# marekrams/tnac4o

Hardware: AMD Instinct MI355X
Metric: PEPS-contraction ms/sweep, chimera L=2048 chi=64 (boundary-MPS sweep _setup_rhoT) (lower is better)
Workload: dtype f64; 1 GPU; chimera L=2048 (Nx=Ny=16, Nc=8), synthetic couplings seed 20260004, beta=3, chi=64; one sweep = 16 rows of MPO absorb + compress_mps; one step = the sweeps of the 4 lattice rotations of one instance; parallelism=1 GPU: 4 lattice rotations of one instance interleaved on 4 HIP streams, mode=sweep

## Files before the change

include/tnpeps.h:

```cpp
#ifndef TNPEPS_H
#define TNPEPS_H
#include <stdint.h>

#ifdef __cplusplus
extern "C" {
#endif

int tn_version(void);
int tn_build_id(char* buf, int n);
int tn_stream_create_masked(const uint32_t* mask_host, int nwords, void** stream_out);
int tn_stream_destroy(void* stream);
int tn_last_error(char* buf, int n);

int tn_gemm(int64_t M, int64_t N, int64_t K, double alpha, const double* A, int64_t rsa, int64_t csa,
            const double* B, int64_t rsb, int64_t csb, double beta, double* C, int64_t rsc, int64_t csc,
            int64_t batch, int64_t bsa, int64_t bsb, int64_t bsc, void* ws, int64_t ws_bytes, void* stream);
int64_t tn_gemm_ws_bytes(int64_t M, int64_t N, int64_t K, int64_t batch);

int tn_factor_products_eligible(int64_t Z, int64_t I, int64_t J, int64_t K1, int64_t N, int64_t M, int first_batched);
int64_t tn_factor_products_ws_bytes(int64_t Z, int64_t I, int64_t J, int64_t K1, int64_t N, int first_batched);
int tn_factor_products(int64_t Z, int64_t I, int64_t J, int64_t K1, int64_t N, int64_t Mhi, int64_t Mlo, const double* P, int64_t pz,
                       int64_t pi, int64_t pk, const double* X, int64_t xk, int64_t xj, int64_t xn, const double* W, int64_t wm,
                       int64_t wq, double* Out, int64_t oz, int64_t ohi, int64_t olo, int64_t on, int first_batched, void* ws,
                       int64_t ws_bytes, void* stream);

int tn_absorb(const double* A, const double* W, double* out, int64_t Dl, int64_t pold, int64_t Dr, int64_t ba,
              int64_t po, int64_t bb, int64_t pi, int hconj, int64_t batch, int64_t bsA, int64_t bsW, int64_t bsOut,
              void* stream);

int tn_qr(double* A, int64_t rs, int64_t cs, int64_t m, int64_t n, double* Q, int64_t qrs, int64_t qcs, double* R,
          int64_t rrs, int64_t rcs, int nb, double rank_tol, int64_t* keff_host, void* ws, int64_t ws_bytes, void* stream);
int64_t tn_qr_ws_bytes(int64_t m, int64_t n, int nb);
int64_t tn_panel_orth_ws_bytes(int64_t nrows, int b);
int tn_panel_orth(const double* X, int64_t rs, int64_t cs, int64_t nrows, int b, double* Y, int64_t yrs, int64_t ycs, int method,
                  int* state9_host, double* dev_host, void* ws, int64_t ws_bytes, void* stream);
int tn_panel_stats(uint64_t* out16_host, int reset);
int tn_panel_stats_stream(uint64_t* out16_host, int reset, void* stream);
int tn_smallqr_stats(uint64_t* out4_host, int reset, void* stream);
int tn_fused_timeouts(int* count_host, void* stream);
int tn_qr_batched(double* A, int64_t rs, int64_t cs, int64_t m, int64_t n, double* Q, int64_t qrs, int64_t qcs, double* R,
// ... 198 lines not shown
```

tnac4o_amd/_lib.py:

```python
import ctypes as C
import os
import subprocess

HERE = os.path.dirname(os.path.abspath(__file__))
LIB_PATH = os.path.join(HERE, 'libtnpeps.so')
CSRC = os.path.join(HERE, 'csrc')
SOURCES = ['api.hip', 'gemm_f64.hip', 'rank_update.hip', 'factor_products.hip', 'small.hip', 'qr.hip', 'svd.hip', 'absorb.hip', 'misc.hip', 'beam.hip', 'prof.hip', 'cholqr.hip', 'smallqr.hip', 'fused.hip', 'peps.hip', 'env.hip', 'batch.hip', 'site.hip', 'chain.hip', 'beamsearch.hip', 'marginal.hip', 'sampler.hip', 'overlap.hip', 'relax.hip', 'exchange.hip', 'temper.hip', 'anneal.hip', 'rng.hip', 'droplets.hip', 'linkage.hip', 'lines.hip']

_i64, _f64, _int, _ptr = C.c_int64, C.c_double, C.c_int, C.c_void_p

SIGNATURES = {
    'tn_version': (_int, []),
    'tn_last_error': (_int, [C.c_char_p, _int]),
    'tn_build_id': (_int, [C.c_char_p, _int]),
    'tn_stream_create_masked': (_int, [C.POINTER(C.c_uint32), _int, C.POINTER(_ptr)]),
    'tn_stream_destroy': (_int, [_ptr]),
    'tn_gemm': (_int, [_i64, _i64, _i64, _f64, _ptr, _i64, _i64, _ptr, _i64, _i64, _f64, _ptr, _i64, _i64,
                       _i64, _i64, _i64, _i64, _ptr, _i64, _ptr]),
    'tn_gemm_ws_bytes': (_i64, [_i64, _i64, _i64, _i64]),
    'tn_factor_products_eligible': (_int, [_i64] * 6 + [_int]),
    'tn_factor_products_ws_bytes': (_i64, [_i64] * 5 + [_int]),
    'tn_factor_products': (_int, [_i64] * 7 + [_ptr, _i64, _i64, _i64, _ptr, _i64, _i64, _i64, _ptr, _i64, _i64, _ptr, _i64, _i64, _i64, _i64,
                                  _int, _ptr, _i64, _ptr]),
    'tn_absorb': (_int, [_ptr, _ptr, _ptr, _i64, _i64, _i64, _i64, _i64, _i64, _i64, _int, _i64, _i64, _i64, _i64, _ptr]),
    'tn_qr': (_int, [_ptr, _i64, _i64, _i64, _i64, _ptr, _i64, _i64, _ptr, _i64, _i64, _int, _f64, C.POINTER(_i64), _ptr, _i64,
              _ptr]),
    'tn_qr_ws_bytes': (_i64, [_i64, _i64, _int]),
    'tn_panel_orth_ws_bytes': (_i64, [_i64, _int]),
    'tn_panel_orth': (_int, [_ptr, _i64, _i64, _i64, _int, _ptr, _i64, _i64, _int, C.POINTER(_int), C.POINTER(_f64), _ptr, _i64, _ptr]),
    'tn_panel_stats': (_int, [C.POINTER(C.c_uint64), _int]),
    'tn_panel_stats_stream': (_int, [C.POINTER(C.c_uint64), _int, _ptr]),
    'tn_smallqr_stats': (_int, [C.POINTER(C.c_uint64), _int, _ptr]),
    'tn_fused_timeouts': (_int, [C.POINTER(_int), _ptr]),
    'tn_qr_batched': (_int, [_ptr, _i64, _i64, _i64, _i64, _ptr, _i64, _i64, _ptr, _i64, _i64, _int, _f64, C.POINTER(_i64), _i64, _i64, _i64,
                      _i64, _ptr, _i64, _ptr, C.POINTER(_ptr), _int]),
    'tn_svd_trunc': (_int, [_ptr, _i64, _i64, _i64, _i64, _i64, _f64, _ptr, _i64, _i64, _ptr, _ptr, _i64, _i64,
                            C.POINTER(_i64), C.POINTER(_f64), C.POINTER(_int), C.POINTER(_int), _ptr, _i64, _ptr]),
    'tn_svdvals': (_int, [_ptr, _i64, _i64, _i64, _i64, C.POINTER(_f64), C.POINTER(_int), C.POINTER(_int), _ptr, _i64,
                          _ptr]),
    'tn_svd_ws_bytes': (_i64, [_i64, _i64, _int]),
    'tn_svdvals_async': (_int, [_ptr, _i64, _i64, _i64, _i64, _ptr, _ptr]),
    'tn_svdvals_small_batched': (_int, [_ptr, _i64, _ptr, _ptr, _ptr]),
# ... 146 lines not shown
        objs = list(ex.map(one, SOURCES))
    cmd = [hipcc, '--offload-arch=gfx950', '-shared', '-fPIC', '-Wl,--no-undefined'] + os.environ.get('TN_EXTRA_HIPCC_FLAGS', '').split() + ['-o', LIB_PATH] + objs
    if verbose:
        print(' '.join(cmd), flush=True)
    subprocess.run(cmd, check=True)
    return LIB_PATH


def _stale(L):
    buf = C.create_string_buffer(64)
    L.tn_build_id.restype, L.tn_build_id.argtypes = _int, [C.c_char_p, _int]
    L.tn_build_id(buf, 64)
    return buf.value.decode() != source_hash()


SHORT_CALLS = ('tn_gemm', 'tn_gemm_ws_bytes', 'tn_qr_ws_bytes', 'tn_svd_ws_bytes', 'tn_absorb', 'tn_nfactor', 'tn_scale_by',
               'tn_normalize_pow2', 'tn_scale_phys', 'tn_calc_pn', 'tn_sample_pn', 'tn_score_pn', 'tn_nfactor_batched', 'tn_env_rr_batched', 'tn_env_rl_batched',
               'tn_balance', 'tn_merge_groups', 'tn_svdvals_async', 'tn_rar', 'tn_rar_ws_bytes', 'tn_env_mix', 'tn_env_mix_ws_bytes',
               'tn_apply_truncation', 'tn_apply_truncation_ws_bytes', 'tn_site_qr_ws_bytes', 'tn_gram_weights', 'tn_argsort_desc', 'tn_weighted_sum', 'tn_rows_norm2', 'tn_gather_scale_rows', 'tn_peps_factor', 'tn_mpo_from_factor', 'tn_env3', 'tn_env3_ws_bytes',
               'tn_cluster_marginal', 'tn_cluster_marginal_ws_bytes', 'tn_cluster_bond_marginal', 'tn_cluster_bond_marginal_ws_bytes',
               'tn_mpo_from_factor_ops', 'tn_env3_stack', 'tn_env3_stack_ws_bytes', 'tn_stack_cell_law', 'tn_stack_cell_law_ws_bytes',
               'tn_last_error')
_lib = None
ABI_VERSION = 25


def lib():
    global _lib
    if _lib is None:
        if not os.path.exists(LIB_PATH):
            raise RuntimeError('libtnpeps.so not found at %s: run `python -c "import __graft_entry__ as g; g.build()"` '
                               '(the HIP library is the only backend; there is no CPU fallback)' % LIB_PATH)
        L = C.CDLL(LIB_PATH)
        L.tn_version.restype = _int
        if not hasattr(L, 'tn_build_id') or (_stale(L) and not os.environ.get('TN_ALLOW_STALE_LIB')):
            raise RuntimeError('libtnpeps.so was built from other sources than csrc/*.hip + include/tnpeps.h in this tree: '
                               'rebuild it with `python -c "import __graft_entry__ as g; g.build()"` -- a stale library can '
                               'disagree with the ctypes signatures declared here')
        if L.tn_version() != ABI_VERSION:
            raise RuntimeError('libtnpeps.so implements C-ABI version %d, this package binds version %d: rebuild the library'
                               % (L.tn_version(), ABI_VERSION))
        if os.environ.get('TN_PYDLL', '1') != '0':
            P = C.PyDLL(LIB_PATH)
            for name in SHORT_CALLS:
                setattr(L, name, getattr(P, name))
            L._pydll = P
        for name, (res, args) in SIGNATURES.items():
# ... 16 lines not shown
```

tnac4o_amd/csrc/api.hip:

```cpp
#include <stdarg.h>

#include "../../include/tnpeps.h"
#include "common.h"

namespace tn {

static thread_local char g_err[512] = "";

void set_error(const char* fmt, ...) {
    va_list ap;
    va_start(ap, fmt);
    vsnprintf(g_err, sizeof(g_err), fmt, ap);
    va_end(ap);
}
const char* get_error() { return g_err; }

}

using namespace tn;
#define ST ((hipStream_t)stream)

extern "C" {

int tn_version(void) { return 25; }

#ifndef TN_SRC_HASH
#define TN_SRC_HASH "unknown"
#endif
int tn_build_id(char* buf, int n) {
    const char* e = TN_SRC_HASH;
    const int len = (int)strlen(e);
    if (buf && n > 0) {
        const int c = len < n - 1 ? len : n - 1;
        memcpy(buf, e, c);
        buf[c] = 0;
    }
    return len;
}

void tn_profile_enable(unsigned mask) { prof_set_mask(mask); }
void tn_profile_reset(void) { prof_reset(); }
void tn_profile_sample(unsigned every) { prof_set_sample(every); }
int tn_profile_get(int family, uint64_t* calls_host, double* ms_host, double* flops_host, double* bytes_host) {
    TN_CHECK_ARG(family >= 0 && family < PROF_NFAM, "unknown kernel family");
    TN_CHECK_ARG(calls_host && ms_host && flops_host && bytes_host, "null output");
    prof_get(-1, family, calls_host, ms_host, flops_host, bytes_host);
    return 0;
// ... 20 lines not shown
    const hipError_t e = hipStreamDestroy((hipStream_t)stream);
    return e == hipSuccess ? 0 : hip_fail(e, "hipStreamDestroy");
}

int tn_last_error(char* buf, int n) {
    const char* e = get_error();
    int len = (int)strlen(e);
    if (buf && n > 0) {
        int c = len < n - 1 ? len : n - 1;
        memcpy(buf, e, c);
        buf[c] = 0;
    }
    return len;
}

int tn_gemm(int64_t M, int64_t N, int64_t K, double alpha, const double* A, int64_t rsa, int64_t csa, const double* B,
            int64_t rsb, int64_t csb, double beta, double* C, int64_t rsc, int64_t csc, int64_t batch, int64_t bsa,
            int64_t bsb, int64_t bsc, void* ws, int64_t ws_bytes, void* stream) {
    TN_CHECK_ARG(M >= 0 && N >= 0 && K >= 0 && batch >= 0, "negative dimension");
    TN_CHECK_ARG(A && B && C, "null operand");
    return gemm(ST, M, N, K, alpha, A, rsa, csa, B, rsb, csb, beta, C, rsc, csc, batch, bsa, bsb, bsc, (double*)ws, ws_bytes);
}
int64_t tn_gemm_ws_bytes(int64_t M, int64_t N, int64_t K, int64_t batch) { return gemm_ws_bytes(M, N, K, batch); }

int tn_factor_products_eligible(int64_t Z, int64_t I, int64_t J, int64_t K1, int64_t N, int64_t M, int first_batched) {
    return factor_products_fits(Z, I, J, K1, N, M) && (first_batched || gemm_ws_bytes(Z * I, J * N, K1, 1) == 0) ? 1 : 0;
}
static int64_t factor_products_layout(char* base, int64_t Z, int64_t I, int64_t J, int64_t K1, int64_t N, int first_batched, double** S,
                                      double** gw, int64_t* gw_bytes) {
    WsCarve c{base};
    *gw_bytes = first_batched ? 0 : gemm_ws_bytes(Z * I, J * N, K1, 1);
    *S = c.take<double>(Z * I * J * N * 8);
    *gw = c.take<double>(*gw_bytes);
    return c.total();
}
int64_t tn_factor_products_ws_bytes(int64_t Z, int64_t I, int64_t J, int64_t K1, int64_t N, int first_batched) {
    double* S; double* gw; int64_t gb;
    return factor_products_layout(nullptr, Z, I, J, K1, N, first_batched, &S, &gw, &gb);
}
int tn_factor_products(int64_t Z, int64_t I, int64_t J, int64_t K1, int64_t N, int64_t Mhi, int64_t Mlo, const double* P, int64_t pz,
                       int64_t pi, int64_t pk, const double* X, int64_t xk, int64_t xj, int64_t xn, const double* W, int64_t wm,
                       int64_t wq, double* Out, int64_t oz, int64_t ohi, int64_t olo, int64_t on, int first_batched, void* ws,
                       int64_t ws_bytes, void* stream) {
    TN_CHECK_ARG(Z >= 1 && I >= 1 && J >= 1 && K1 >= 1 && N >= 1 && Mhi >= 1 && Mlo >= 1, "non-positive dimension");
    TN_CHECK_ARG(P && X && W && Out, "null operand");
    TN_CHECK_ARG((Z == 1 || pz == I * pi) && (first_batched || J == 1 || xj == N * xn), "the first product needs pz = I pi, and unbatched xj = N xn");
// ... 276 lines not shown
```

tnac4o_amd/csrc/common.h:

```cpp
#pragma once
#include <hip/hip_runtime.h>
#include <stdint.h>
#include <stdio.h>
#include <stdlib.h>
#include <string.h>

namespace tn {

void set_error(const char* fmt, ...);
const char* get_error();

inline int hip_fail(hipError_t e, const char* what) {
    set_error("%s: %s", what, hipGetErrorString(e));
    return (int)e > 0 ? (int)e : 1;
}

#define TN_CHECK_ARG(cond, msg)                \
    do {                                       \
        if (!(cond)) {                         \
            tn::set_error("%s: %s", __func__, msg); \
            return -1;                         \
        }                                      \
    } while (0)

// ... 63 lines not shown
void prof_note_qr(int64_t m, int64_t n, int64_t batch);
void prof_note_svd(int64_t k, int64_t n, int sweeps);
void prof_note_svdvals(int64_t k, int64_t n);
int prof_phase(int phase);
struct ProfPhase {
    int prev;
    explicit ProfPhase(int ph) : prev(prof_phase(ph)) {}
    ~ProfPhase() { prof_phase(prev); }
};
#define TN_PROF_LAUNCH(st, fam, launch) do { prof_begin(st, fam); launch; prof_end(st, fam, 0.0, 0.0); } while (0)
void prof_set_mask(unsigned mask);
void prof_set_sample(unsigned n);
void prof_reset();
void prof_get(int phase, int fam, uint64_t* calls, double* ms, double* flops, double* bytes);

struct Mat {
    double* p;
    int64_t rs, cs;
};
static inline Mat mat(double* p, int64_t rs, int64_t cs) { return Mat{p, rs, cs}; }
static inline Mat sub(Mat a, int64_t i, int64_t j) { return Mat{a.p + i * a.rs + j * a.cs, a.rs, a.cs}; }
static inline Mat tr(Mat a) { return Mat{a.p, a.cs, a.rs}; }

int gemm(hipStream_t st, int64_t M, int64_t N, int64_t K, double alpha, const double* A, int64_t rsa, int64_t csa,
         const double* B, int64_t rsb, int64_t csb, double beta, double* C, int64_t rsc, int64_t csc,
         int64_t batch = 1, int64_t bsa = 0, int64_t bsb = 0, int64_t bsc = 0, double* ws = nullptr,
         int64_t ws_bytes = 0);
int64_t gemm_ws_bytes(int64_t M, int64_t N, int64_t K, int64_t batch);
struct GemmExtra {
    const int* pairs = nullptr;
    const int* skip = nullptr;
    int pw = 0, mapA = 0, mapB = 0, mapC = 0;
    int force_splitk = 0;
    bool raw_partials = false;
    int* splitk_used = nullptr;
};
int gemm_forced_split(int64_t K, int s, int64_t* kchunk);
int gemm_ex(hipStream_t st, int64_t M, int64_t N, int64_t K, double alpha, const double* A, int64_t rsa, int64_t csa,
            const double* B, int64_t rsb, int64_t csb, double beta, double* C, int64_t rsc, int64_t csc, int64_t batch,
            int64_t bsa, int64_t bsb, int64_t bsc, double* ws, int64_t ws_bytes, const GemmExtra* x);

static inline int gemm(hipStream_t st, int64_t M, int64_t N, int64_t K, double alpha, Mat A, Mat B, double beta, Mat C,
                       double* ws = nullptr, int64_t ws_bytes = 0) {
    return gemm(st, M, N, K, alpha, A.p, A.rs, A.cs, B.p, B.rs, B.cs, beta, C.p, C.rs, C.cs, 1, 0, 0, 0, ws, ws_bytes);
}
int gemm_prof_family(int64_t M, int64_t N, int64_t K, int64_t rsc, int64_t csc);

int rank_update(hipStream_t st, int64_t m, int64_t n, int b, const double* W, int64_t wrs, int64_t wcs, const double* X, int64_t xrs,
                int64_t xcs, double* C, int64_t rsc, int64_t csc, const int* active);
static inline int rank_update(hipStream_t st, int64_t m, int64_t n, int b, Mat W, Mat X, Mat C, const int* active = nullptr) {
    return rank_update(st, m, n, b, W.p, W.rs, W.cs, X.p, X.rs, X.cs, C.p, C.rs, C.cs, active);
}

struct FactorProducts {
    int64_t Z, I, J, K1, N, Mhi, Mlo;
    const double* P; int64_t pz, pi, pk;
    const double* X; int64_t xk, xj, xn;
    const double* W; int64_t wm, wq;
    double* Out; int64_t oz, ohi, olo, on;
};
bool factor_products_fits(int64_t Z, int64_t I, int64_t J, int64_t K1, int64_t N, int64_t M);
inline bool factor_products_on() { return env_flag_on("TN_FACTOR_FUSED"); }
int factor_products(hipStream_t st, const FactorProducts& f);

constexpr int NBMAX = 64;

int gram_partial(hipStream_t st, const double* X, int64_t vs, int64_t es, int64_t L, int nvec, int w, const int* pairs,
                 int ngroups, int nchunk, double* part);
// ... 159 lines not shown
```

tnac4o_amd/csrc/factor_products.hip:

```cpp
#include "common.h"

namespace tn {

namespace {

typedef double d4 __attribute__((ext_vector_type(4)));

constexpr int FP_NC = 64;
constexpr int FP_QMAX = 256;
constexpr int FP_IMAX = 16;
constexpr int FP_K1MAX = 64;
constexpr int FP_THREADS = 512, FP_WAVES = FP_THREADS / 64;
constexpr int FP_SLAB = 32 * FP_WAVES;

struct FacP {
    const double* P;
    const double* X;
    const double* W;
    double* Out;
    int Z, I, J, K1, N, M, Mlo, chunks;
    int64_t pz, pi, pk, xk, xj, xn, wm, wq, oz, ohi, olo, on;
};

__device__ __forceinline__ int fp_sidx(int q, int c) { return q * FP_NC + (c ^ ((q & 1) << 4)); }

__device__ __forceinline__ double fp_keep(double v, bool keep) {
    long long m = keep ? -1ll : 0ll;
    asm volatile("" : "+v"(m));
    return __longlong_as_double(__double_as_longlong(v) & m);
}

template <int KS>
__device__ __forceinline__ void fp_stage1(const FacP& g, double* S, const int z, const int n0, const int nb, const int wave, const int lr, const int lk) {
    constexpr int KG = 4 * KS;
    double p[KG];
    {
        const double* Pz = g.P + (int64_t)z * g.pz + (int64_t)min(lr, g.I - 1) * g.pi;
#pragma unroll
        for (int kk = 0; kk < KG; ++kk) {
            const int k = kk * 4 + lk;
            const double v = Pz[(int64_t)min(k, g.K1 - 1) * g.pk];
            p[kk] = fp_keep(v, lr < g.I && k < g.K1);
        }
    }
    const int units = g.J * nb;
    auto load = [&](double (&b)[KG], const int u) {
        const int uc = min(u, units - 1), j = uc / nb, cb = uc - j * nb, n = n0 + cb * 16 + lr;
        const double* Xp = g.X + (int64_t)j * g.xj + (int64_t)min(n, g.N - 1) * g.xn;
#pragma unroll
        for (int kk = 0; kk < KG; ++kk) {
            const int k = kk * 4 + lk;
            const double v = Xp[(int64_t)min(k, g.K1 - 1) * g.xk];
            b[kk] = fp_keep(v, n < g.N && k < g.K1);
// ... 147 lines not shown
```

tnac4o_amd/csrc/gemm_f64.hip:

```cpp
#include <stdlib.h>

#include <algorithm>
#include <map>
#include <mutex>
#include <tuple>
#include <vector>

#include "common.h"

namespace tn {

typedef double d4 __attribute__((ext_vector_type(4)));

struct GemmP {
    const double* A;
    const double* B;
    double* C;
    int64_t M, N, K;
    int64_t rsa, csa, rsb, csb, rsc, csc;
    int64_t bsa, bsb, bsc;
    double alpha, beta;
    int splitk;
    int64_t kchunk;
    double* ws;
    int tiles_m, tiles_n;
    const int* pairs;
    const int* skip;
    int pw, mapA, mapB, mapC;
};

constexpr int BK = 16;

template <int BM, int BN, int BKT, bool AKFAST, bool BKFAST, bool MAPPED>
__global__ __launch_bounds__(256, (BM == 128 && BN == 128 && BKT == 16) ? 2 : 1) void gemm_kernel(GemmP g) {
    constexpr int BK = BKT;
    constexpr int PA = BM + 16, PB = BN + 16;
    constexpr int WM = BM / 2, WN = BN / 2, TM = WM / 16, TN = WN / 16;
    constexpr int EA = BM * BK / 256, EB = BN * BK / 256;
    __shared__ double As[2][BK * PA];
    __shared__ double Bs[2][BK * PB];

    const int tid = threadIdx.x, lane = tid & 63, wave = tid >> 6;
    const int wm = wave >> 1, wn = wave & 1;
    int bid = blockIdx.x;
    {
        const int nwg = gridDim.x, q = nwg / 8, r = nwg % 8, xcd = bid % 8, loc = bid / 8;
        bid = (xcd < r ? xcd * (q + 1) : r * (q + 1) + (xcd - r) * q) + loc;
    }
    const int tm0 = (bid / g.tiles_n) * BM, tn0 = (bid % g.tiles_n) * BN;
    const int nsk = g.splitk < 0 ? 1 : g.splitk;
    const int zb = blockIdx.z / nsk, zs = blockIdx.z % nsk;
    if (g.skip && g.skip[zb] == 0) return;
    int blk0 = 0, blk1 = 0;
    if (MAPPED && g.pairs) { blk0 = g.pairs[2 * zb]; blk1 = g.pairs[2 * zb + 1]; }
    auto remap = [&](int64_t v) -> int64_t { return v < g.pw ? (int64_t)blk0 * g.pw + v : (int64_t)blk1 * g.pw + (v - g.pw); };
    const double* A = g.A + zb * g.bsa;
    const double* B = g.B + zb * g.bsb;
    const int64_t k_lo = zs * g.kchunk;
    const int64_t k_hi = (k_lo + g.kchunk < g.K) ? k_lo + g.kchunk : g.K;

    constexpr int DM = AKFAST ? 256 / BK : 0, DKA = AKFAST ? 0 : 256 / BM;
    constexpr int DN = BKFAST ? 256 / BK : 0, DKB = BKFAST ? 0 : 256 / BN;
    const int m0 = AKFAST ? tid / BK : tid % BM, kA0 = AKFAST ? tid % BK : tid / BM;
    const int n0 = BKFAST ? tid / BK : tid % BN, kB0 = BKFAST ? tid % BK : tid / BN;
    const int64_t offA0 = (int64_t)(tm0 + m0) * g.rsa + (int64_t)kA0 * g.csa, stepA = (int64_t)DM * g.rsa + (int64_t)DKA * g.csa;
    const int64_t offB0 = (int64_t)(tn0 + n0) * g.csb + (int64_t)kB0 * g.rsb, stepB = (int64_t)DN * g.csb + (int64_t)DKB * g.rsb;

    double ra[EA], rb[EB];
    auto load_tiles = [&](int64_t k0) {
        if constexpr (!MAPPED) {
            const double* Ak = A + k0 * g.csa + offA0;
            const double* Bk = B + k0 * g.rsb + offB0;
#pragma unroll
            for (int e = 0; e < EA; ++e)
                ra[e] = (tm0 + m0 + e * DM < g.M && k0 + kA0 + e * DKA < k_hi) ? Ak[e * stepA] : 0.0;
#pragma unroll
            for (int e = 0; e < EB; ++e)
                rb[e] = (tn0 + n0 + e * DN < g.N && k0 + kB0 + e * DKB < k_hi) ? Bk[e * stepB] : 0.0;
        } else {
#pragma unroll
            for (int e = 0; e < EA; ++e) {
                const int64_t gm = tm0 + m0 + e * DM, gk = k0 + kA0 + e * DKA;
                ra[e] = (gm < g.M && gk < k_hi) ? A[(g.mapA ? remap(gm) : gm) * g.rsa + gk * g.csa] : 0.0;
            }
#pragma unroll
            for (int e = 0; e < EB; ++e) {
                const int64_t gn = tn0 + n0 + e * DN, gk = k0 + kB0 + e * DKB;
                rb[e] = (gn < g.N && gk < k_hi) ? B[(g.mapB == 1 ? remap(gk) : gk) * g.rsb + (g.mapB == 2 ? remap(gn) : gn) * g.csb] : 0.0;
            }
        }
    };
    auto store_tiles = [&](int stage) {
#pragma unroll
        for (int e = 0; e < EA; ++e) {
            const int m = m0 + e * DM, k = kA0 + e * DKA;
            As[stage][k * PA + (m ^ k)] = ra[e];
        }
#pragma unroll
        for (int e = 0; e < EB; ++e) {
            const int n = n0 + e * DN, k = kB0 + e * DKB;
            Bs[stage][k * PB + (n ^ k)] = rb[e];
        }
    };

    d4 acc[TM][TN];
#pragma unroll
    for (int i = 0; i < TM; ++i)
#pragma unroll
        for (int j = 0; j < TN; ++j) acc[i][j] = d4{0.0, 0.0, 0.0, 0.0};

    const int lr = lane & 15, lk = lane >> 4;
    int cur = 0;
    if (k_lo < k_hi) {
        load_tiles(k_lo);
        store_tiles(0);
    }
    __syncthreads();
    for (int64_t k0 = k_lo; k0 < k_hi; k0 += BK) {
        const bool more = k0 + BK < k_hi;
        if (more) load_tiles(k0 + BK);
        const double* Ac = As[cur];
        const double* Bc = Bs[cur];
#pragma unroll
        for (int kk = 0; kk < BK / 4; ++kk) {
            const int k = kk * 4 + lk;
            double a[TM], b[TN];
#pragma unroll
            for (int i = 0; i < TM; ++i) a[i] = Ac[k * PA + ((wm * WM + i * 16 + lr) ^ k)];
#pragma unroll
            for (int j = 0; j < TN; ++j) b[j] = Bc[k * PB + ((wn * WN + j * 16 + lr) ^ k)];
#pragma unroll
            for (int i = 0; i < TM; ++i)
#pragma unroll
                for (int j = 0; j < TN; ++j)
                    acc[i][j] = __builtin_amdgcn_mfma_f64_16x16x4f64(a[i], b[j], acc[i][j], 0, 0, 0);
        }
        if (more) store_tiles(cur ^ 1);
        __syncthreads();
        cur ^= 1;
    }

    if (g.splitk > 1 || g.splitk < 0) {
        double* W = g.ws + (int64_t)blockIdx.z * g.M * g.N;
#pragma unroll
        for (int i = 0; i < TM; ++i)
#pragma unroll
            for (int j = 0; j < TN; ++j)
#pragma unroll
                for (int r = 0; r < 4; ++r) {
                    const int64_t row = tm0 + wm * WM + i * 16 + lk + 4 * r, col = tn0 + wn * WN + j * 16 + lr;
                    if (row < g.M && col < g.N) W[row * g.N + col] = acc[i][j][r];
                }
    } else {
        double* C = g.C + zb * g.bsc;
        const bool hb = g.beta != 0.0;
        if (hb) {
            double cv[2][TN][4];
            auto fetch = [&](int i, int buf) {
#pragma unroll
                for (int j = 0; j < TN; ++j)
#pragma unroll
                    for (int r = 0; r < 4; ++r) {
// ... 11 lines not shown
                    for (int r = 0; r < 4; ++r) {
                        const int64_t row = tm0 + wm * WM + i * 16 + lk + 4 * r, col = tn0 + wn * WN + j * 16 + lr;
                        if (row < g.M && col < g.N) {
                            double v = g.alpha * acc[i][j][r];
                            v += g.beta * cv[i & 1][j][r];
                            C[((MAPPED && g.mapC) ? remap(row) : row) * g.rsc + col * g.csc] = v;
                        }
                    }
            }
        } else {
#pragma unroll
            for (int i = 0; i < TM; ++i)
#pragma unroll
                for (int j = 0; j < TN; ++j)
#pragma unroll
                    for (int r = 0; r < 4; ++r) {
                        const int64_t row = tm0 + wm * WM + i * 16 + lk + 4 * r, col = tn0 + wn * WN + j * 16 + lr;
                        if (row < g.M && col < g.N) C[((MAPPED && g.mapC) ? remap(row) : row) * g.rsc + col * g.csc] = g.alpha * acc[i][j][r];
                    }
        }
    }
}

__global__ __launch_bounds__(256) void splitk_reduce_kernel(GemmP g) {
    const int64_t mn = g.M * g.N;
    const int64_t e = (int64_t)blockIdx.x * 256 + threadIdx.x;
    const int zb = blockIdx.y;
    if (e >= mn) return;
    if (g.skip && g.skip[zb] == 0) return;
    const double* W = g.ws + (int64_t)zb * g.splitk * mn + e;
    double s = 0.0;
    int k = 0;
    for (; k + 8 <= g.splitk; k += 8) {
        double v[8];
#pragma unroll
        for (int u = 0; u < 8; ++u) v[u] = W[(int64_t)(k + u) * mn];
#pragma unroll
        for (int u = 0; u < 8; ++u) s += v[u];
    }
    for (; k < g.splitk; ++k) s += W[(int64_t)k * mn];
    const int64_t row = e / g.N, col = e % g.N;
    double* c = g.C + zb * g.bsc + row * g.rsc + col * g.csc;
    double v = g.alpha * s;
    if (g.beta != 0.0) v += g.beta * *c;
    *c = v;
}

template <int BM, int BN, int BKT>
static void launch_tile(hipStream_t st, const GemmP& g, dim3 grid, bool ak, bool bk) {
    if constexpr (BM == 64 && BN == 64) {
        if (g.pairs) {
            if (ak && bk) hipLaunchKernelGGL((gemm_kernel<BM, BN, BKT, true, true, true>), grid, dim3(256), 0, st, g);
            else if (ak) hipLaunchKernelGGL((gemm_kernel<BM, BN, BKT, true, false, true>), grid, dim3(256), 0, st, g);
            else if (bk) hipLaunchKernelGGL((gemm_kernel<BM, BN, BKT, false, true, true>), grid, dim3(256), 0, st, g);
            else hipLaunchKernelGGL((gemm_kernel<BM, BN, BKT, false, false, true>), grid, dim3(256), 0, st, g);
            return;
        }
    }
    if (ak && bk) hipLaunchKernelGGL((gemm_kernel<BM, BN, BKT, true, true, false>), grid, dim3(256), 0, st, g);
    else if (ak) hipLaunchKernelGGL((gemm_kernel<BM, BN, BKT, true, false, false>), grid, dim3(256), 0, st, g);
    else if (bk) hipLaunchKernelGGL((gemm_kernel<BM, BN, BKT, false, true, false>), grid, dim3(256), 0, st, g);
    else hipLaunchKernelGGL((gemm_kernel<BM, BN, BKT, false, false, false>), grid, dim3(256), 0, st, g);
}

struct GemmPlan { int bm, bn, s; };
static GemmPlan plan_gemm(int64_t M, int64_t N, int64_t K, int64_t batch) {
    static const int64_t small_work = (int64_t)1 << env_int("TN_GEMM_SMALLWORK_LOG2", 30);
    static const int big_tiles = env_int("TN_GEMM_BIGTILES", 1 << 30);
    static const int target_wg = env_int("TN_GEMM_TARGETWG", 256);
    static const int min_chunk = env_int("TN_GEMM_MINCHUNK", 32);
    static const int smax = env_int("TN_GEMM_SMAX", 64);
    static const int bigsplit_wgs = env_int("TN_GEMM_BIGSPLIT_WGS", 192), bigsplit_target = env_int("TN_GEMM_BIGSPLIT_TARGET", 512);
    const bool small = (double)M * (double)N * (double)K * (double)batch < (double)small_work;
    GemmPlan p;
    if (M > 64 && N > 64) {
        const bool big = !small || cdiv(M, 128) * cdiv(N, 128) * batch >= big_tiles;
        p.bm = p.bn = big ? 128 : 64;
    } else if (N <= 32 && M > 64) { p.bm = 128; p.bn = 32; }
    else if (M <= 32 && N > 64) { p.bm = 32; p.bn = 128; }
    else { p.bm = 64; p.bn = 64; }
    const int64_t wgs = cdiv(M, p.bm) * cdiv(N, p.bn) * batch;
    p.s = 1;
    if (small) {
        if (wgs < target_wg * 3 / 4 && K >= 2 * min_chunk) {
            int64_t s = wgs <= 16 ? smax : cdiv(target_wg, wgs);
// ... 128 lines not shown
        const int64_t fit = ws ? ws_bytes / (batch * M * N * 8) : 0;
        if (fit < s) s = fit < 2 ? 1 : (int)fit;
    }
    const bool raw = x && x->raw_partials;
    TN_CHECK_ARG(!raw || ws != nullptr, "raw partials need a workspace");
    g.splitk = s = gemm_forced_split(K, s, &g.kchunk);
    if (raw && s == 1) g.splitk = -1;
    if (x && x->splitk_used) *x->splitk_used = s;
    if (batch * s > 65535) {
        TN_CHECK_ARG(x == nullptr && s <= 65535, "batch*splitk exceeds grid.z");
        const int64_t cb = 65535 / s;
        for (int64_t b0 = 0; b0 < batch; b0 += cb) {
            const int64_t nbt = batch - b0 < cb ? batch - b0 : cb;
            const int rc = gemm_ex_impl(st, M, N, K, alpha, A + b0 * bsa, rsa, csa, B + b0 * bsb, rsb, csb, beta, C + b0 * bsc, rsc, csc,
                                        nbt, bsa, bsb, bsc, ws, ws_bytes, nullptr);
            if (rc) return rc;
        }
        return 0;
    }
    const bool ak = (csa == 1 && rsa != 1), bk = (rsb == 1 && csb != 1);
    dim3 grid(g.tiles_m * g.tiles_n, 1, (unsigned)(batch * s));
    const int fam = tile_family(pl);
    prof_begin(st, fam);
    if (bm == 128 && bn == 128) launch_tile<128, 128, 16>(st, g, grid, ak, bk);
    else if (bm == 128 && bn == 32) launch_tile<128, 32, 16>(st, g, grid, ak, bk);
    else if (bm == 32 && bn == 128) launch_tile<32, 128, 16>(st, g, grid, ak, bk);
    else launch_tile<64, 64, 16>(st, g, grid, ak, bk);
    TN_CHECK_LAUNCH("gemm_kernel");
    prof_end(st, fam, 2.0 * M * N * K * batch, 8.0 * batch * ((double)M * K + (double)K * N + (double)M * N));
    if (s > 1 && !raw) {
        dim3 rg((unsigned)cdiv(M * N, 256), (unsigned)batch);
        prof_begin(st, PROF_SPLITK_REDUCE);
        hipLaunchKernelGGL(splitk_reduce_kernel, rg, dim3(256), 0, st, g);
        TN_CHECK_LAUNCH("splitk_reduce_kernel");
        prof_end(st, PROF_SPLITK_REDUCE, (double)s * M * N * batch, 8.0 * batch * ((double)s + 1.0) * M * N);
    }
    return 0;
}

}
```

Before: 358.2 ms/sweep.

## Restructure GEMM tile loads with clamped offset walker and configurable prefetch depth

```diff
diff --git a/include/tnpeps.h b/include/tnpeps.h
--- a/include/tnpeps.h
+++ b/include/tnpeps.h
@@ -16,6 +16,12 @@
             const double* B, int64_t rsb, int64_t csb, double beta, double* C, int64_t rsc, int64_t csc,
             int64_t batch, int64_t bsa, int64_t bsb, int64_t bsc, void* ws, int64_t ws_bytes, void* stream);
 int64_t tn_gemm_ws_bytes(int64_t M, int64_t N, int64_t K, int64_t batch);
+int tn_gemm_ex(int64_t M, int64_t N, int64_t K, double alpha, const double* A, int64_t rsa, int64_t csa,
+               const double* B, int64_t rsb, int64_t csb, double beta, double* C, int64_t rsc, int64_t csc,
+               int64_t batch, int64_t bsa, int64_t bsb, int64_t bsc, void* ws, int64_t ws_bytes, const int* skip,
+               int force_splitk, void* stream);
+int64_t tn_gemm_walk_probe(int bmn, int kfast, int64_t MN, int64_t K, int64_t kchunk, int depth, int64_t sx, int64_t sk,
+                           int64_t* off, unsigned char* keep, int64_t cap);
 
 int tn_factor_products_eligible(int64_t Z, int64_t I, int64_t J, int64_t K1, int64_t N, int64_t M, int first_batched);
 int64_t tn_factor_products_ws_bytes(int64_t Z, int64_t I, int64_t J, int64_t K1, int64_t N, int first_batched);
diff --git a/tnac4o_amd/_lib.py b/tnac4o_amd/_lib.py
--- a/tnac4o_amd/_lib.py
+++ b/tnac4o_amd/_lib.py
@@ -18,6 +18,9 @@
     'tn_gemm': (_int, [_i64, _i64, _i64, _f64, _ptr, _i64, _i64, _ptr, _i64, _i64, _f64, _ptr, _i64, _i64,
                        _i64, _i64, _i64, _i64, _ptr, _i64, _ptr]),
     'tn_gemm_ws_bytes': (_i64, [_i64, _i64, _i64, _i64]),
+    'tn_gemm_ex': (_int, [_i64, _i64, _i64, _f64, _ptr, _i64, _i64, _ptr, _i64, _i64, _f64, _ptr, _i64, _i64,
+                          _i64, _i64, _i64, _i64, _ptr, _i64, _ptr, _int, _ptr]),
+    'tn_gemm_walk_probe': (_i64, [_int, _int, _i64, _i64, _i64, _int, _i64, _i64, C.POINTER(_i64), C.POINTER(C.c_ubyte), _i64]),
     'tn_factor_products_eligible': (_int, [_i64] * 6 + [_int]),
     'tn_factor_products_ws_bytes': (_i64, [_i64] * 5 + [_int]),
     'tn_factor_products': (_int, [_i64] * 7 + [_ptr, _i64, _i64, _i64, _ptr, _i64, _i64, _i64, _ptr, _i64, _i64, _ptr, _i64, _i64, _i64, _i64,
@@ -210,7 +213,7 @@
                'tn_mpo_from_factor_ops', 'tn_env3_stack', 'tn_env3_stack_ws_bytes', 'tn_stack_cell_law', 'tn_stack_cell_law_ws_bytes',
                'tn_last_error')
 _lib = None
-ABI_VERSION = 25
+ABI_VERSION = 26
 
 
 def lib():
diff --git a/tnac4o_amd/csrc/api.hip b/tnac4o_amd/csrc/api.hip
--- a/tnac4o_amd/csrc/api.hip
+++ b/tnac4o_amd/csrc/api.hip
@@ -22,7 +22,7 @@
 
 extern "C" {
 
-int tn_version(void) { return 25; }
+int tn_version(void) { return 26; }
 
 #ifndef TN_SRC_HASH
 #define TN_SRC_HASH "unknown"
@@ -89,6 +89,20 @@
     return gemm(ST, M, N, K, alpha, A, rsa, csa, B, rsb, csb, beta, C, rsc, csc, batch, bsa, bsb, bsc, (double*)ws, ws_bytes);
 }
 int64_t tn_gemm_ws_bytes(int64_t M, int64_t N, int64_t K, int64_t batch) { return gemm_ws_bytes(M, N, K, batch); }
+int tn_gemm_ex(int64_t M, int64_t N, int64_t K, double alpha, const double* A, int64_t rsa, int64_t csa, const double* B,
+               int64_t rsb, int64_t csb, double beta, double* C, int64_t rsc, int64_t csc, int64_t batch, int64_t bsa,
+               int64_t bsb, int64_t bsc, void* ws, int64_t ws_bytes, const int* skip, int force_splitk, void* stream) {
+    TN_CHECK_ARG(M >= 0 && N >= 0 && K >= 0 && batch >= 0 && force_splitk >= 0, "negative dimension");
+    TN_CHECK_ARG(A && B && C, "null operand");
+    GemmExtra x;
+    x.skip = skip;
+    x.force_splitk = force_splitk;
+    return gemm_ex(ST, M, N, K, alpha, A, rsa, csa, B, rsb, csb, beta, C, rsc, csc, batch, bsa, bsb, bsc, (double*)ws, ws_bytes, &x);
+}
+int64_t tn_gemm_walk_probe(int bmn, int kfast, int64_t MN, int64_t K, int64_t kchunk, int depth, int64_t sx, int64_t sk, int64_t* off,
+                           unsigned char* keep, int64_t cap) {
+    return gemm_walk_probe(bmn, kfast, MN, K, kchunk, depth, sx, sk, off, keep, cap);
+}
 
 int tn_factor_products_eligible(int64_t Z, int64_t I, int64_t J, int64_t K1, int64_t N, int64_t M, int first_batched) {
     return factor_products_fits(Z, I, J, K1, N, M) && (first_batched || gemm_ws_bytes(Z * I, J * N, K1, 1) == 0) ? 1 : 0;
diff --git a/tnac4o_amd/csrc/common.h b/tnac4o_amd/csrc/common.h
--- a/tnac4o_amd/csrc/common.h
+++ b/tnac4o_amd/csrc/common.h
@@ -109,6 +109,13 @@
 static inline Mat sub(Mat a, int64_t i, int64_t j) { return Mat{a.p + i * a.rs + j * a.cs, a.rs, a.cs}; }
 static inline Mat tr(Mat a) { return Mat{a.p, a.cs, a.rs}; }
 
+__device__ __forceinline__ double fp_keep(double v, bool keep) {
+    long long m = keep ? -1ll : 0ll;
+    asm volatile("" : "+v"(m));
+    return __longlong_as_double(__double_as_longlong(v) & m);
+}
+__host__ __device__ inline int64_t clamp_offset(int i, int hi, int64_t off_i, int64_t off_hi) { return i > hi ? off_hi : off_i; }
+
 int gemm(hipStream_t st, int64_t M, int64_t N, int64_t K, double alpha, const double* A, int64_t rsa, int64_t csa,
          const double* B, int64_t rsb, int64_t csb, double beta, double* C, int64_t rsc, int64_t csc,
          int64_t batch = 1, int64_t bsa = 0, int64_t bsb = 0, int64_t bsc = 0, double* ws = nullptr,
@@ -131,6 +138,8 @@
                        double* ws = nullptr, int64_t ws_bytes = 0) {
     return gemm(st, M, N, K, alpha, A.p, A.rs, A.cs, B.p, B.rs, B.cs, beta, C.p, C.rs, C.cs, 1, 0, 0, 0, ws, ws_bytes);
 }
+int64_t gemm_walk_probe(int bmn, int kfast, int64_t MN, int64_t K, int64_t kchunk, int depth, int64_t sx, int64_t sk, int64_t* off,
+                        unsigned char* keep, int64_t cap);
 int gemm_prof_family(int64_t M, int64_t N, int64_t K, int64_t rsc, int64_t csc);
 
 int rank_update(hipStream_t st, int64_t m, int64_t n, int b, const double* W, int64_t wrs, int64_t wcs, const double* X, int64_t xrs,
diff --git a/tnac4o_amd/csrc/factor_products.hip b/tnac4o_amd/csrc/factor_products.hip
--- a/tnac4o_amd/csrc/factor_products.hip
+++ b/tnac4o_amd/csrc/factor_products.hip
@@ -23,12 +23,6 @@
 };
 
 __device__ __forceinline__ int fp_sidx(int q, int c) { return q * FP_NC + (c ^ ((q & 1) << 4)); }
-
-__device__ __forceinline__ double fp_keep(double v, bool keep) {
-    long long m = keep ? -1ll : 0ll;
-    asm volatile("" : "+v"(m));
-    return __longlong_as_double(__double_as_longlong(v) & m);
-}
 
 template <int KS>
 __device__ __forceinline__ void fp_stage1(const FacP& g, double* S, const int z, const int n0, const int nb, const int wave, const int lr, const int lk) {
diff --git a/tnac4o_amd/csrc/gemm_f64.hip b/tnac4o_amd/csrc/gemm_f64.hip
--- a/tnac4o_amd/csrc/gemm_f64.hip
+++ b/tnac4o_amd/csrc/gemm_f64.hip
@@ -31,12 +31,58 @@
 
 constexpr int BK = 16;
 
-template <int BM, int BN, int BKT, bool AKFAST, bool BKFAST, bool MAPPED>
+template <int BMN, int BKT, bool KFAST>
+struct TileWalk {
+    static constexpr int E = BMN * BKT / 256;
+    static constexpr int DX = KFAST ? 256 / BKT : 0, DK = KFAST ? 0 : 256 / BMN;
+    int kk0, xrem;
+    bool xfull;
+    int64_t kt, kmax;
+    int64_t run;
+    int64_t at_kmax;
+    int64_t dox, dok, stepk;
+    static __host__ __device__ int x0(int tid) { return KFAST ? tid / BKT : tid % BMN; }
+    __host__ __device__ void init(int tid, int64_t t0, int64_t MN, int64_t k_lo, int64_t k_hi, int64_t sx, int64_t sk) {
+        const int64_t xr = MN - 1 - (t0 + x0(tid)), x = xr < 0 ? MN - 1 : t0 + x0(tid);
+        kk0 = KFAST ? tid % BKT : tid / BMN;
+        xrem = (int)(xr < -1 ? -1 : (xr > BMN ? BMN : xr));
+        xfull = t0 + BMN <= MN;
+        kt = k_lo; kmax = k_hi - 1;
+        dox = DX * sx; dok = DK * sk; stepk = BKT * sk;
+        run = x * sx + (k_lo + kk0) * sk;
+        at_kmax = KFAST ? 0 : x * sx + kmax * sk;
+    }
+    __host__ __device__ void advance() { kt += BKT; run += stepk; }
+    __host__ __device__ int krem(int64_t k0) const { const int64_t r = kmax - k0; return (int)(r < -1 ? -1 : (r > BKT ? BKT : r)); }
+    __host__ __device__ bool inner(int kr) const { return xfull && kr >= BKT - 1; }
+    __host__ __device__ bool keep(int e, int kr) const { return e * DX <= xrem && kk0 <= kr - e * DK; }
+    __host__ __device__ void offsets(int64_t (&off)[E]) const {
+        const int kr = krem(kt);
+        if (inner(kr)) {
+            off[0] = run;
+#pragma unroll
+            for (int e = 1; e < E; ++e) off[e] = off[e - 1] + (KFAST ? dox : dok);
+        } else if (KFAST) {
+            const int64_t over = kt + kk0 - kmax;
+            off[0] = run - (over > 0 ? over : 0);
+#pragma unroll
+            for (int e = 1; e < E; ++e) off[e] = off[e - 1] + clamp_offset(e * DX, xrem, dox, 0);
+        } else {
+#pragma unroll
+            for (int e = 0; e < E; ++e) off[e] = clamp_offset(kk0, kr - e * DK, run + e * dok, at_kmax);
+        }
+    }
+};
+
+template <int BM, int BN, int BKT, bool AKFAST, bool BKFAST, bool MAPPED, int PF>
 __global__ __launch_bounds__(256, (BM == 128 && BN == 128 && BKT == 16) ? 2 : 1) void gemm_kernel(GemmP g) {
+    static_assert(!MAPPED || PF == 1, "the block-pair indirection keeps its guarded loads and the one-tile schedule");
     constexpr int BK = BKT;
     constexpr int PA = BM + 16, PB = BN + 16;
     constexpr int WM = BM / 2, WN = BN / 2, TM = WM / 16, TN = WN / 16;
-    constexpr int EA = BM * BK / 256, EB = BN * BK / 256;
+    using WalkA = TileWalk<BM, BK, AKFAST>;
+    using WalkB = TileWalk<BN, BK, BKFAST>;
+    constexpr int EA = WalkA::E, EB = WalkB::E;
     __shared__ double As[2][BK * PA];
     __shared__ double Bs[2][BK * PB];
 
@@ -59,47 +105,67 @@
     const int64_t k_lo = zs * g.kchunk;
     const int64_t k_hi = (k_lo + g.kchunk < g.K) ? k_lo + g.kchunk : g.K;
 
-    constexpr int DM = AKFAST ? 256 / BK : 0, DKA = AKFAST ? 0 : 256 / BM;
-    constexpr int DN = BKFAST ? 256 / BK : 0, DKB = BKFAST ? 0 : 256 / BN;
+    constexpr int DM = WalkA::DX, DKA = WalkA::DK, DN = WalkB::DX, DKB = WalkB::DK;
     const int m0 = AKFAST ? tid / BK : tid % BM, kA0 = AKFAST ? tid % BK : tid / BM;
     const int n0 = BKFAST ? tid / BK : tid % BN, kB0 = BKFAST ? tid % BK : tid / BN;
-    const int64_t offA0 = (int64_t)(tm0 + m0) * g.rsa + (int64_t)kA0 * g.csa, stepA = (int64_t)DM * g.rsa + (int64_t)DKA * g.csa;
-    const int64_t offB0 = (int64_t)(tn0 + n0) * g.csb + (int64_t)kB0 * g.rsb, stepB = (int64_t)DN * g.csb + (int64_t)DKB * g.rsb;
-
-    double ra[EA], rb[EB];
-    auto load_tiles = [&](int64_t k0) {
+    WalkA wa;
+    WalkB wb;
+    if (k_lo < k_hi) {
+        wa.init(tid, tm0, g.M, k_lo, k_hi, g.rsa, g.csa);
+        wb.init(tid, tn0, g.N, k_lo, k_hi, g.csb, g.rsb);
+    }
+
+    double ra[PF][EA], rb[PF][EB];
+    auto load_tiles = [&](double (&qa)[EA], double (&qb)[EB], int64_t k0) {
         if constexpr (!MAPPED) {
-            const double* Ak = A + k0 * g.csa + offA0;
-            const double* Bk = B + k0 * g.rsb + offB0;
-#pragma unroll
-            for (int e = 0; e < EA; ++e)
-                ra[e] = (tm0 + m0 + e * DM < g.M && k0 + kA0 + e * DKA < k_hi) ? Ak[e * stepA] : 0.0;
-#pragma unroll
-            for (int e = 0; e < EB; ++e)
-                rb[e] = (tn0 + n0 + e * DN < g.N && k0 + kB0 + e * DKB < k_hi) ? Bk[e * stepB] : 0.0;
+            if constexpr (AKFAST) asm volatile("" : "+v"(wa.dox));
+            if constexpr (BKFAST) asm volatile("" : "+v"(wb.dox));
+            int64_t oa[EA], ob[EB];
+            wa.offsets(oa);
+            wb.offsets(ob);
+#pragma unroll
+            for (int e = 0; e < EA; ++e) qa[e] = A[oa[e]];
+#pragma unroll
+            for (int e = 0; e < EB; ++e) qb[e] = B[ob[e]];
+            wa.advance();
+            wb.advance();
         } else {
 #pragma unroll
             for (int e = 0; e < EA; ++e) {
                 const int64_t gm = tm0 + m0 + e * DM, gk = k0 + kA0 + e * DKA;
-                ra[e] = (gm < g.M && gk < k_hi) ? A[(g.mapA ? remap(gm) : gm) * g.rsa + gk * g.csa] : 0.0;
+                qa[e] = (gm < g.M && gk < k_hi) ? A[(g.mapA ? remap(gm) : gm) * g.rsa + gk * g.csa] : 0.0;
             }
 #pragma unroll
             for (int e = 0; e < EB; ++e) {
                 const int64_t gn = tn0 + n0 + e * DN, gk = k0 + kB0 + e * DKB;
-                rb[e] = (gn < g.N && gk < k_hi) ? B[(g.mapB == 1 ? remap(gk) : gk) * g.rsb + (g.mapB == 2 ? remap(gn) : gn) * g.csb] : 0.0;
+                qb[e] = (gn < g.N && gk < k_hi) ? B[(g.mapB == 1 ? remap(gk) : gk) * g.rsb + (g.mapB == 2 ? remap(gn) : gn) * g.csb] : 0.0;
             }
         }
     };
-    auto store_tiles = [&](int stage) {
+    auto store_tiles = [&](int stage, const double (&qa)[EA], const double (&qb)[EB], int64_t k0) {
+        double va[EA], vb[EB];
+#pragma unroll
+        for (int e = 0; e < EA; ++e) va[e] = qa[e];
+#pragma unroll
+        for (int e = 0; e < EB; ++e) vb[e] = qb[e];
+        if constexpr (!MAPPED) {
+            const int kr = wa.krem(k0);
+            if (!(wa.inner(kr) && wb.inner(kr))) {
+#pragma unroll
+                for (int e = 0; e < EA; ++e) va[e] = fp_keep(va[e], wa.keep(e, kr));
+#pragma unroll
+                for (int e = 0; e < EB; ++e) vb[e] = fp_keep(vb[e], wb.keep(e, kr));
+            }
+        }
 #pragma unroll
         for (int e = 0; e < EA; ++e) {
             const int m = m0 + e * DM, k = kA0 + e * DKA;
-            As[stage][k * PA + (m ^ k)] = ra[e];
+            As[stage][k * PA + (m ^ k)] = va[e];
         }
 #pragma unroll
         for (int e = 0; e < EB; ++e) {
             const int n = n0 + e * DN, k = kB0 + e * DKB;
-            Bs[stage][k * PB + (n ^ k)] = rb[e];
+            Bs[stage][k * PB + (n ^ k)] = vb[e];
         }
     };
 
@@ -112,32 +178,44 @@
     const int lr = lane & 15, lk = lane >> 4;
     int cur = 0;
     if (k_lo < k_hi) {
-        load_tiles(k_lo);
-        store_tiles(0);
-    }
-    __syncthreads();
-    for (int64_t k0 = k_lo; k0 < k_hi; k0 += BK) {
-        const bool more = k0 + BK < k_hi;
-        if (more) load_tiles(k0 + BK);
-        const double* Ac = As[cur];
-        const double* Bc = Bs[cur];
-#pragma unroll
-        for (int kk = 0; kk < BK / 4; ++kk) {
-            const int k = kk * 4 + lk;
-            double a[TM], b[TN];
-#pragma unroll
-            for (int i = 0; i < TM; ++i) a[i] = Ac[k * PA + ((wm * WM + i * 16 + lr) ^ k)];
-#pragma unroll
-            for (int j = 0; j < TN; ++j) b[j] = Bc[k * PB + ((wn * WN + j * 16 + lr) ^ k)];
-#pragma unroll
-            for (int i = 0; i < TM; ++i)
-#pragma unroll
-                for (int j = 0; j < TN; ++j)
-                    acc[i][j] = __builtin_amdgcn_mfma_f64_16x16x4f64(a[i], b[j], acc[i][j], 0, 0, 0);
-        }
-        if (more) store_tiles(cur ^ 1);
+        int64_t kl = k_lo, k0 = k_lo;
+#pragma unroll
+        for (int s = 0; s < PF; ++s) {
+            load_tiles(ra[s], rb[s], kl);
+            kl += BK;
+        }
+        store_tiles(0, ra[0], rb[0], k_lo);
         __syncthreads();
-        cur ^= 1;
+        for (bool more = true; more;) {
+#pragma unroll
+            for (int s = 0; s < PF; ++s) {
+                load_tiles(ra[s], rb[s], kl);
+                kl += BK;
+                __builtin_amdgcn_sched_barrier(0);
+                const double* Ac = As[cur];
+                const double* Bc = Bs[cur];
+#pragma unroll
+                for (int kk = 0; kk < BK / 4; ++kk) {
+                    const int k = kk * 4 + lk, sw = lr ^ k;
+                    double a[TM], b[TN];
+#pragma unroll
+                    for (int i = 0; i < TM; ++i) a[i] = Ac[k * PA + wm * WM + i * 16 + sw];
+#pragma unroll
+                    for (int j = 0; j < TN; ++j) b[j] = Bc[k * PB + wn * WN + j * 16 + sw];
+#pragma unroll
+                    for (int i = 0; i < TM; ++i)
+#pragma unroll
+                        for (int j = 0; j < TN; ++j)
+                            acc[i][j] = __builtin_amdgcn_mfma_f64_16x16x4f64(a[i], b[j], acc[i][j], 0, 0, 0);
+                }
+                __builtin_amdgcn_sched_barrier(0);
+                k0 += BK;
+                if (k0 >= k_hi) { more = false; break; }
+                store_tiles(cur ^ 1, ra[(s + 1) % PF], rb[(s + 1) % PF], k0);
+                __syncthreads();
+                cur ^= 1;
+            }
+        }
     }
 
     if (g.splitk > 1 || g.splitk < 0) {
@@ -195,6 +273,44 @@
     }
 }
 
+template <int BMN, bool KFAST>
+static int64_t walk_probe(int64_t MN, int64_t K, int64_t kchunk, int depth, int64_t sx, int64_t sk, int64_t* off, unsigned char* keep, int64_t cap) {
+    using Walk = TileWalk<BMN, BK, KFAST>;
+    int64_t n = 0;
+    for (int64_t t0 = 0; t0 < MN; t0 += BMN)
+        for (int64_t k_lo = 0; k_lo < K; k_lo += kchunk) {
+            const int64_t k_hi = k_lo + kchunk < K ? k_lo + kchunk : K;
+            const int64_t requests = cdiv(k_hi - k_lo, BK) + depth;
+            if (n + requests * 256 * Walk::E > cap) return -1;
+            for (int tid = 0; tid < 256; ++tid) {
+                Walk w;
+                w.init(tid, t0, MN, k_lo, k_hi, sx, sk);
+                for (int64_t j = 0; j < requests; ++j) {
+                    int64_t o[Walk::E];
+                    w.offsets(o);
+                    for (int e = 0; e < Walk::E; ++e) {
+                        const int64_t at = n + (j * 256 + tid) * Walk::E + e;
+                        off[at] = o[e];
+                        keep[at] = w.keep(e, w.krem(w.kt)) ? 1 : 0;
+                    }
+                    w.advance();
+                }
+            }
+            n += requests * 256 * Walk::E;
+        }
+    return n;
+}
+
+int64_t gemm_walk_probe(int bmn, int kfast, int64_t MN, int64_t K, int64_t kchunk, int depth, int64_t sx, int64_t sk, int64_t* off,
+                        unsigned char* keep, int64_t cap) {
+    if (MN <= 0 || K <= 0 || kchunk <= 0 || kchunk % BK || depth < 1 || depth > 4 || !off || !keep || (kfast && sk != 1)) return -1;
+    if (bmn == 32) return kfast ? walk_probe<32, true>(MN, K, kchunk, depth, sx, sk, off, keep, cap) : walk_probe<32, false>(MN, K, kchunk, depth, sx, sk, off, keep, cap);
+    if (bmn == 64) return kfast ? walk_probe<64, true>(MN, K, kchunk, depth, sx, sk, off, keep, cap) : walk_probe<64, false>(MN, K, kchunk, depth, sx, sk, off, keep, cap);
+    if (bmn == 128) return kfast ? walk_probe<128, true>(MN, K, kchunk, depth, sx, sk, off, keep, cap) : walk_probe<128, false>(MN, K, kchunk, depth, sx, sk, off, keep, cap);
+    return -1;
+}
+
+template <int R>
 __global__ __launch_bounds__(256) void splitk_reduce_kernel(GemmP g) {
     const int64_t mn = g.M * g.N;
     const int64_t e = (int64_t)blockIdx.x * 256 + threadIdx.x;
@@ -203,15 +319,13 @@
     if (g.skip && g.skip[zb] == 0) return;
     const double* W = g.ws + (int64_t)zb * g.splitk * mn + e;
     double s = 0.0;
-    int k = 0;
-    for (; k + 8 <= g.splitk; k += 8) {
-        double v[8];
-#pragma unroll
-        for (int u = 0; u < 8; ++u) v[u] = W[(int64_t)(k + u) * mn];
-#pragma unroll
-        for (int u = 0; u < 8; ++u) s += v[u];
-    }
-    for (; k < g.splitk; ++k) s += W[(int64_t)k * mn];
+    for (int k = 0; k < g.splitk; k += R) {
+        double v[R];
+#pragma unroll
+        for (int u = 0; u < R; ++u) v[u] = W[(int64_t)min(k + u, g.splitk - 1) * mn];
+#pragma unroll
+        for (int u = 0; u < R; ++u) s += fp_keep(v[u], k + u < g.splitk);
+    }
     const int64_t row = e / g.N, col = e % g.N;
     double* c = g.C + zb * g.bsc + row * g.rsc + col * g.csc;
     double v = g.alpha * s;
@@ -219,21 +333,46 @@
     *c = v;
 }
 
-template <int BM, int BN, int BKT>
+static void launch_reduce(hipStream_t st, const GemmP& g, dim3 grid) {
+    if (g.splitk <= 8) hipLaunchKernelGGL(splitk_reduce_kernel<8>, grid, dim3(256), 0, st, g);
+    else if (g.splitk <= 16) hipLaunchKernelGGL(splitk_reduce_kernel<16>, grid, dim3(256), 0, st, g);
+    else if (g.splitk <= 32) hipLaunchKernelGGL(splitk_reduce_kernel<32>, grid, dim3(256), 0, st, g);
+    else hipLaunchKernelGGL(splitk_reduce_kernel<64>, grid, dim3(256), 0, st, g);
+}
+
+constexpr int PF_128x128 = 1, PF_128x32 = 1, PF_32x128 = 1, PF_64x64 = 1;
+
+template <int BM, int BN, int BKT, int PF>
 static void launch_tile(hipStream_t st, const GemmP& g, dim3 grid, bool ak, bool bk) {
+    if (ak && bk) hipLaunchKernelGGL((gemm_kernel<BM, BN, BKT, true, true, false, PF>), grid, dim3(256), 0, st, g);
+    else if (ak) hipLaunchKernelGGL((gemm_kernel<BM, BN, BKT, true, false, false, PF>), grid, dim3(256), 0, st, g);
+    else if (bk) hipLaunchKernelGGL((gemm_kernel<BM, BN, BKT, false, true, false, PF>), grid, dim3(256), 0, st, g);
+    else hipLaunchKernelGGL((gemm_kernel<BM, BN, BKT, false, false, false, PF>), grid, dim3(256), 0, st, g);
+}
+
+template <int BM, int BN, int DEPTH>
+static void launch_class(hipStream_t st, const GemmP& g, dim3 grid, bool ak, bool bk) {
     if constexpr (BM == 64 && BN == 64) {
         if (g.pairs) {
-            if (ak && bk) hipLaunchKernelGGL((gemm_kernel<BM, BN, BKT, true, true, true>), grid, dim3(256), 0, st, g);
-            else if (ak) hipLaunchKernelGGL((gemm_kernel<BM, BN, BKT, true, false, true>), grid, dim3(256), 0, st, g);
-            else if (bk) hipLaunchKernelGGL((gemm_kernel<BM, BN, BKT, false, true, true>), grid, dim3(256), 0, st, g);
-            else hipLaunchKernelGGL((gemm_kernel<BM, BN, BKT, false, false, true>), grid, dim3(256), 0, st, g);
+            if (ak && bk) hipLaunchKernelGGL((gemm_kernel<BM, BN, 16, true, true, true, 1>), grid, dim3(256), 0, st, g);
+            else if (ak) hipLaunchKernelGGL((gemm_kernel<BM, BN, 16, true, false, true, 1>), grid, dim3(256), 0, st, g);
+            else if (bk) hipLaunchKernelGGL((gemm_kernel<BM, BN, 16, false, true, true, 1>), grid, dim3(256), 0, st, g);
+            else hipLaunchKernelGGL((gemm_kernel<BM, BN, 16, false, false, true, 1>), grid, dim3(256), 0, st, g);
             return;
         }
     }
-    if (ak && bk) hipLaunchKernelGGL((gemm_kernel<BM, BN, BKT, true, true, false>), grid, dim3(256), 0, st, g);
-    else if (ak) hipLaunchKernelGGL((gemm_kernel<BM, BN, BKT, true, false, false>), grid, dim3(256), 0, st, g);
-    else if (bk) hipLaunchKernelGGL((gemm_kernel<BM, BN, BKT, false, true, false>), grid, dim3(256), 0, st, g);
-    else hipLaunchKernelGGL((gemm_kernel<BM, BN, BKT, false, false, false>), grid, dim3(256), 0, st, g);
+    const char* e = env_str("TN_GEMM_PREFETCH");
+    const int v = e ? atoi(e) : -1;
+#ifdef TN_GEMM_ALL_DEPTHS
+    const int d = v < 0 ? DEPTH : v;
+    if (d == 2) return launch_tile<BM, BN, 16, 2>(st, g, grid, ak, bk);
+    if (d == 3) return launch_tile<BM, BN, 16, 3>(st, g, grid, ak, bk);
+    if (d >= 4) return launch_tile<BM, BN, 16, 4>(st, g, grid, ak, bk);
+#else
+    if constexpr (DEPTH > 1)
+        if (v != 0) return launch_tile<BM, BN, 16, DEPTH>(st, g, grid, ak, bk);
+#endif
+    launch_tile<BM, BN, 16, 1>(st, g, grid, ak, bk);
 }
 
 struct GemmPlan { int bm, bn, s; };
@@ -408,16 +547,16 @@
     dim3 grid(g.tiles_m * g.tiles_n, 1, (unsigned)(batch * s));
     const int fam = tile_family(pl);
     prof_begin(st, fam);
-    if (bm == 128 && bn == 128) launch_tile<128, 128, 16>(st, g, grid, ak, bk);
-    else if (bm == 128 && bn == 32) launch_tile<128, 32, 16>(st, g, grid, ak, bk);
-    else if (bm == 32 && bn == 128) launch_tile<32, 128, 16>(st, g, grid, ak, bk);
-    else launch_tile<64, 64, 16>(st, g, grid, ak, bk);
+    if (bm == 128 && bn == 128) launch_class<128, 128, PF_128x128>(st, g, grid, ak, bk);
+    else if (bm == 128 && bn == 32) launch_class<128, 32, PF_128x32>(st, g, grid, ak, bk);
+    else if (bm == 32 && bn == 128) launch_class<32, 128, PF_32x128>(st, g, grid, ak, bk);
+    else launch_class<64, 64, PF_64x64>(st, g, grid, ak, bk);
     TN_CHECK_LAUNCH("gemm_kernel");
     prof_end(st, fam, 2.0 * M * N * K * batch, 8.0 * batch * ((double)M * K + (double)K * N + (double)M * N));
     if (s > 1 && !raw) {
         dim3 rg((unsigned)cdiv(M * N, 256), (unsigned)batch);
         prof_begin(st, PROF_SPLITK_REDUCE);
-        hipLaunchKernelGGL(splitk_reduce_kernel, rg, dim3(256), 0, st, g);
+        launch_reduce(st, g, rg);
         TN_CHECK_LAUNCH("splitk_reduce_kernel");
         prof_end(st, PROF_SPLITK_REDUCE, (double)s * M * N * batch, 8.0 * batch * ((double)s + 1.0) * M * N);
     }
```

Result: slower. 362.0 ms/sweep (+1.0%).
